# Banus/pano360

Measured on AMD Instinct MI355X. Metric: blended megapixels/sec (multiband), higher is better.
Workload: dtype f32; 1 GPU; cfg3: 32 synthetic 3840x2160 frames per image set, spherical warp + multiband blend L=5, native resolution (MAX_RESOLUTION uncapped); frames=32

## Files before the change

include/pano360.h:

```cpp
#ifndef PANO360_H
#define PANO360_H

#include <stddef.h>
#include <stdint.h>

#ifdef __cplusplus
extern "C" {
#endif

#define PANO_OK 0
#define PANO_EINVAL (-1)
#define PANO_EHIP (-2)
#define PANO_ELIMIT (-3)
#define PANO_ESOLVE (-4)

#define PANO_MAX_TAPS 129
#define PANO_MAX_LEVELS 8
#define PANO_TAP_LEAD 7
#define PANO_TAP_PAD 40
#ifndef PANO_INTERIOR_BLOCK
#define PANO_INTERIOR_BLOCK 4
#endif
#ifndef PANO_MEDIAN_KEEP
#define PANO_MEDIAN_KEEP 32
// ... 84 lines not shown
                        const double *tan_p, const float *lut255, const double *hat_x,
                        const double *hat_y, int gx0, int gy0, int pw, int ph,
                        float *planes, uint8_t *mask, float *map_x, float *map_y);

int pano_warp_windows(pano_ctx *ctx, const pano_camera *cams, const pano_patch *patches,
                      int n, int max_vw, int max_vh, const double *sin_t,
                      const double *cos_t, const double *tan_p, const float *lut,
                      int lut_stride, const uint8_t *need);

int pano_ownership(pano_ctx *ctx, const pano_patch *patches, int n, int H, int W,
                   int16_t *owner, uint8_t *valid);

int pano_ownership_cameras(pano_ctx *ctx, const pano_camera *cams, int n, int H, int W,
                           int xs0, int xs1, const double *sin_t, const double *cos_t,
                           const double *tan_p, int16_t *owner, uint8_t *valid);

int pano_owned_regions(pano_ctx *ctx, const int16_t *owner, int H, int W, int xs0, int xs1,
                       int n, int min_gap, int max_spans, uint8_t *marks,
                       int32_t *regions);

int pano_ownership_regions(pano_ctx *ctx, const pano_camera *cams, int n, int H, int W,
                           int xs0, int xs1, const double *sin_t, const double *cos_t,
                           const double *tan_p, int16_t *owner, uint8_t *valid,
                           int min_gap, int max_spans, uint8_t *marks, int32_t *regions);

int pano_blur_tile_grid(const pano_ctx *ctx);
int pano_blur_tiles(pano_ctx *ctx, const pano_patch *patches, int n, int max_aw,
                    int max_ah, int W, int radius, const uint8_t *interior,
                    uint8_t *tile_flags, uint8_t *warp_need);
int pano_multiband_blur_prepare(pano_ctx *ctx, const pano_patch *patches, int n,
// ... 436 lines not shown
```

pano360_amd/_lib.py:

```python
import ctypes as C
import os
import subprocess

import numpy as np

_HERE = os.path.dirname(os.path.abspath(__file__))
LIB_PATH = os.environ.get("PANO_LIB") or os.path.join(_HERE, "libpano360_hip.so")

MAX_TAPS = 129
MAX_LEVELS = 8
TAP_LEAD = 7
TAP_PAD = 40
OPT_BLUR_KERNEL, OPT_OWN_PRUNE, OPT_BLUR_SEGMENTS, OPT_BLUR_LEAN, OPT_STITCH_STREAMS = 0, 1, 2, 3, 4
OPT_STITCH_ASYNC = 5
OPT_BLUR_SEG_LEN = 6
OPT_SIFT_GRAPH = 7
OPT_LEVEL_CLASSES = 8
BLUR_MFMA, BLUR_VALU = 0, 1


class PanoError(RuntimeError):
    """A C-ABI call returned a negative status."""


# ... 190 lines not shown
    "pano_ctx_destroy": (_i, [_vp]),
    "pano_ctx_set_stream": (_i, [_vp, _vp]),
    "pano_ctx_set_option": (_i, [_vp, _i, _i]),
    "pano_ctx_get_option": (_i, [_vp, _i, C.POINTER(C.c_int)]),
    "pano_timing_enable": (_i, [_vp, _i]),
    "pano_kernel_count": (_i, []),
    "pano_kernel_name": (C.c_char_p, [_i]),
    "pano_timing_read": (_i, [_vp, _i, C.POINTER(C.c_double), C.POINTER(C.c_int)]),
    "pano_add_weights": (_i, [_vp, _vp, _i, _i, _vp, _vp, _vp, _vp]),
    "pano_warp_spherical": (_i, [_vp, _vp, _i, _i, _vp, _vp, _vp, _vp, _vp, _vp, _vp, _i, _i, _i,
                                 _i, _vp, _vp, _vp, _vp]),
    "pano_warp_windows": (_i, [_vp, _vp, _vp, _i, _i, _i, _vp, _vp, _vp, _vp, _i, _vp]),
    "pano_blur_tiles": (_i, [_vp, _vp, _i, _i, _i, _i, _i, _vp, _vp, _vp]),
    "pano_ownership": (_i, [_vp, _vp, _i, _i, _i, _vp, _vp]),
    "pano_ownership_cameras": (_i, [_vp, _vp, _i, _i, _i, _i, _i, _vp, _vp, _vp, _vp, _vp]),
    "pano_owned_regions": (_i, [_vp, _vp, _i, _i, _i, _i, _i, _i, _i, _vp, _vp]),
    "pano_ownership_regions": (_i, [_vp, _vp, _i, _i, _i, _i, _i, _vp, _vp, _vp, _vp, _vp,
                                    _i, _i, _vp, _vp]),
    "pano_multiband_blur": (_i, [_vp, _vp, _i, _i, _i, _i, _vp, _i, _vp, C.POINTER(C.c_int), _i,
                                 _vp, _vp]),
    "pano_multiband_blur_prepare": (_i, [_vp, _vp, _i, _i, _i, _i, _vp, _vp]),
    "pano_layout_windows": (_i, [_i, _vp, _i, _i, _vp, _vp, _i, _i, _i, _i, _vp, _i, _vp]),
    "pano_layout_place": (_i, [_vp, _i, _vp, _vp, _vp]),
    "pano_interior_map": (_i, [_vp, _vp, _i, _i, _i, _i, _i, _vp, _vp]),
    "pano_interior_classes": (_i, [_vp, _vp, _i, _i, _i, _i, _vp, _i, _vp, _vp, _vp]),
    "pano_multiband_compose": (_i, [_vp, _vp, _i, _i, _i, _i, _i, _i, _vp, _vp, _vp, _vp, _vp, _vp,
                                    _vp, _vp, _vp, _i, _vp, _vp]),
    "pano_blend_cameras": (_i, [_vp, _vp, _i, _i, _i, _i, _i, _i, _vp, _vp, _vp, _vp, _i, _vp,
                                _vp]),
    "pano_blur_tile_grid": (_i, [_vp]),
# ... 226 lines not shown
```

pano360_amd/csrc/api.hip:

```cpp
#include <stdarg.h>
#include <stdio.h>
#include <stdlib.h>
#include <string.h>

#include <vector>

#include "common.h"
#include "layout.h"

static thread_local char g_error[512] = "";

void pano_set_error(const char *fmt, ...) {
    va_list ap;
    va_start(ap, fmt);
    vsnprintf(g_error, sizeof(g_error), fmt, ap);
    va_end(ap);
}

extern "C" const char *pano_version(void) { return "pano360_hip 0.1 (gfx950)"; }

extern "C" const char *pano_last_error(void) { return g_error; }

extern "C" int pano_device_count(void) {
    int n = 0;
// ... 127 lines not shown
    PANO_REQUIRE(ctx, "pano_ctx_set_stream: null context");
    if ((hipStream_t)stream != ctx->stream) stitch_memo_void_geometry(ctx->memo);
    ctx->stream = (hipStream_t)stream;
    return PANO_OK;
}

extern "C" int pano_ctx_set_option(pano_ctx *ctx, int option, int value) {
    PANO_REQUIRE(ctx, "pano_ctx_set_option: null context");
    PANO_REQUIRE(option >= 0 && option < PANO_OPT_COUNT, "pano_ctx_set_option: option %d", option);
    if (option == PANO_OPT_BLUR_KERNEL)
        PANO_REQUIRE(value == PANO_BLUR_MFMA || value == PANO_BLUR_VALU,
                     "pano_ctx_set_option: blur kernel %d", value);
    else if (option == PANO_OPT_STITCH_ASYNC)
        PANO_REQUIRE(value >= 0 && value <= 2, "pano_ctx_set_option: option %d takes 0, 1 or 2", option);
    else if (option == PANO_OPT_OWN_PRUNE)
        PANO_REQUIRE(value >= 0 && value <= 3, "pano_ctx_set_option: option %d takes 0 .. 3", option);
    else if (option == PANO_OPT_BLUR_SEG_LEN)
        PANO_REQUIRE(value == -1 || value == 0 || (value >= 4 && value <= 2047),
                     "pano_ctx_set_option: option %d takes -1, 0 or 4 .. 2047", option);
    else
        PANO_REQUIRE(value == 0 || value == 1, "pano_ctx_set_option: option %d takes 0 or 1", option);
    const bool changed = ctx->opt[option] != value;
    ctx->opt[option] = value;
    ctx->prepared_table = ctx->flags_table = ctx->list_table = nullptr;
    stitch_memo_void_geometry(ctx->memo);
    if (changed && option == PANO_OPT_BLUR_KERNEL) stitch_memo_void_layout(ctx->memo);
    return PANO_OK;
}

extern "C" int pano_ctx_get_option(const pano_ctx *ctx, int option, int *value) {
    PANO_REQUIRE(ctx && value, "pano_ctx_get_option: null pointer");
// ... 199 lines not shown
```

pano360_amd/csrc/blend.hip:

```cpp
#include <stdlib.h>

#include "geom.h"

__global__ __launch_bounds__(256) void ownership_kernel(
    const pano_patch *__restrict__ patches, int n, int H, int W,
    int16_t *__restrict__ owner, uint8_t *__restrict__ valid) {
    const int x = blockIdx.x * 64 + threadIdx.x, y = blockIdx.y * 4 + threadIdx.y;
    if (x >= W || y >= H) return;
    float best = 0.0f;
    int who = -1;
    bool any = false;
    for (int i = 0; i < n; ++i) {
        const pano_patch p = patches[i];
        const int px = x - p.x0, py = y - p.y0;
        if ((unsigned)px >= (unsigned)p.w || (unsigned)py >= (unsigned)p.h) continue;
        const float a = p.planes[3 * (size_t)p.vh * p.vpitch + (size_t)py * p.vpitch + px];
        if (a > best) {
            best = a;
            who = i;
        }
        any |= p.mask[(size_t)py * p.w + px] == 0;
    }
    owner[(size_t)y * W + x] = (int16_t)who;
    valid[(size_t)y * W + x] = any ? 1 : 0;
// ... 396 lines not shown
    const int tid = wave * 64 + lane;
    if (tid < listed) {
        const int *b = s_box[tid];
        if (b[1] >= b[0]) box_merge(boxes + (size_t)box_stride * sh.list[tid], b[0], b[1], b[2], b[3]);
    }
}

#define OW_T 64
#define OW_Q 16
#define OW_CAMS 32
#define OW_QLIST 8
#define OW_ILP 4
#define OW_EVAL (-3)
#define OW_NOBODY (-1)
#define OW_UNOWNED (-2)

#define OW_SUBS 8
#define OW_FN(name) name
#include "own_tile.inc"
#undef OW_FN
#define OW_TH_TALL (OW_Q * OW_SUBS)

template <bool LINEAR, bool PERCAM>
__global__ __launch_bounds__(256) void blend_cameras_kernel(
    const pano_camera *__restrict__ cams, int n, int H, int W, int xs0, int xs1,
    const double *__restrict__ sin_t, const double *__restrict__ cos_t,
    const double *__restrict__ tan_p, const float *__restrict__ lut,
    uint8_t *__restrict__ mosaic, uint8_t *__restrict__ valid) {
    __shared__ CamList sh;
    __shared__ CamPrune pr;
// ... 478 lines not shown
#define MOSAIC_GRID dim3 block(64, 4), grid(ceil_div(W, 64), ceil_div(H, 4))

extern "C" int pano_ownership(pano_ctx *ctx, const pano_patch *patches, int n, int H, int W,
                              int16_t *owner, uint8_t *valid) {
    PANO_ENTER(ctx, "pano_ownership");
    if (int rc = check_table(patches, n, H, W, "pano_ownership")) return rc;
    PANO_REQUIRE(owner && valid, "pano_ownership: null output");
    MOSAIC_GRID;
    PANO_TIMED(PK_OWNERSHIP, (hipStream_t)stream,
               hipLaunchKernelGGL(ownership_kernel, grid, block, 0, (hipStream_t)stream,
                                  patches, n, H, W, owner, valid));
    PANO_LAUNCH_CHECK("ownership_kernel");
    return PANO_OK;
}

extern "C" int pano_ownership_cameras(pano_ctx *ctx, const pano_camera *cams, int n, int H, int W,
                                      int xs0, int xs1, const double *sin_t, const double *cos_t,
                                      const double *tan_p, int16_t *owner, uint8_t *valid) {
    PANO_ENTER(ctx, "pano_ownership_cameras");
    if (int rc = check_table(cams, n, H, W, "pano_ownership_cameras")) return rc;
    PANO_REQUIRE(sin_t && cos_t && tan_p && owner && valid, "pano_ownership_cameras: null pointer");
    if (int rc = check_strip(xs0, xs1, W, "pano_ownership_cameras")) return rc;
    if (xs0 == xs1) return PANO_OK;
    const int prune = ctx->opt[PANO_OPT_OWN_PRUNE];
    dim3 block(64, 4), grid(ceil_div(xs1 - xs0, 64), ceil_div(H, (prune & 2) ? OWN_TILE_ROWS : OW_TH_TALL));
    PANO_TIMED(PK_OWNERSHIP_CAMS, (hipStream_t)stream,
               hipLaunchKernelGGL((prune & 2) ? ownership_cameras_l1_kernel : ownership_cameras_kernel,
                                  grid, block, (prune & 2) ? 0 : own_shared_bytes(n),
                                  (hipStream_t)stream, cams, n, H, W, xs0, xs1, sin_t, cos_t,
                                  tan_p, owner, valid, prune & 1, (int32_t *)nullptr, 0,
                                  (uint8_t *)nullptr));
    PANO_LAUNCH_CHECK("ownership_cameras_kernel");
    return PANO_OK;
}

extern "C" int pano_blend_cameras(pano_ctx *ctx, const pano_camera *cams, int n, int H, int W,
                                  int xs0, int xs1, int linear, const double *sin_t,
                                  const double *cos_t, const double *tan_p, const float *lut,
                                  int lut_stride, uint8_t *mosaic, uint8_t *valid) {
    PANO_ENTER(ctx, "pano_blend_cameras");
    if (int rc = check_fused_blend(cams, n, H, W, xs0, xs1, sin_t, cos_t, tan_p, lut, lut_stride,
                                   mosaic, "pano_blend_cameras")) return rc;
    if (xs0 == xs1) return PANO_OK;
    dim3 block(64, 4), grid(ceil_div(xs1 - xs0, 64), ceil_div(H, 4));
    hipStream_t s = (hipStream_t)stream;
#define BLEND(LIN, PC)                                                                        \
    PANO_TIMED(PK_BLEND_CAMERAS, s,                                                           \
               hipLaunchKernelGGL((blend_cameras_kernel<LIN, PC>), grid, block, 0, s, cams, n, \
// ... 118 lines not shown
                                      int xs0, int xs1, const double *sin_t, const double *cos_t,
                                      const double *tan_p, int16_t *owner, uint8_t *valid,
                                      int min_gap, int max_spans, uint8_t *marks,
                                      int32_t *regions) {
    PANO_ENTER(ctx, "pano_ownership_regions");
    if (int rc = check_table(cams, n, H, W, "pano_ownership_regions")) return rc;
    PANO_REQUIRE(sin_t && cos_t && tan_p && owner && valid && marks && regions,
                 "pano_ownership_regions: null pointer");
    if (int rc = check_strip(xs0, xs1, W, "pano_ownership_regions")) return rc;
    PANO_REQUIRE(max_spans >= 1 && min_gap >= 0, "pano_ownership_regions: bad argument");
    if (n == 0) return PANO_OK;
    hipStream_t s = (hipStream_t)stream;
    const int stride = 5 + 2 * max_spans;
    if (int rc = launch_init_regions(s, regions, n, stride, marks, W)) return rc;
    if (xs0 == xs1) return PANO_OK;
    const int prune = ctx->opt[PANO_OPT_OWN_PRUNE];
    dim3 block(64, 4), grid(ceil_div(xs1 - xs0, 64), ceil_div(H, (prune & 2) ? OWN_TILE_ROWS : OW_TH_TALL));
    PANO_TIMED(PK_OWNERSHIP_CAMS, s,
               hipLaunchKernelGGL((prune & 2) ? ownership_cameras_l1_kernel : ownership_cameras_kernel,
                                  grid, block, (prune & 2) ? 0 : own_shared_bytes(n), s, cams, n, H, W, xs0,
                                  xs1, sin_t, cos_t, tan_p, owner, valid, prune & 1, regions, stride,
                                  marks));
    PANO_LAUNCH_CHECK("ownership_cameras_kernel");
    PANO_TIMED(PK_OWNED_SPANS, s,
               hipLaunchKernelGGL(owned_spans_kernel, dim3(n), dim3(256), 0, s, marks, W, xs0, xs1,
                                  min_gap, max_spans, stride, regions));
    PANO_LAUNCH_CHECK("owned_spans_kernel");
    return PANO_OK;
}

static int interior_map_launch(pano_ctx *ctx, const int16_t *owner, int H, int W, int xs0, int xs1,
                               const int *radii, int n_radii, int16_t *block_owner,
                               uint8_t *interior, uint8_t *classes, const char *who) {
    void *const stream = (void *)ctx->stream;
    PANO_REQUIRE(owner && block_owner && interior && radii, "%s: null pointer", who);
    PANO_REQUIRE(H > 0 && W > 0 && n_radii >= 1 && n_radii < PANO_MAX_LEVELS, "%s: bad argument", who);
    if (int rc = check_strip(xs0, xs1, W, who)) return rc;
    LevelReaches lv = {};
// ... 221 lines not shown
```

pano360_amd/csrc/geom.h:

```cpp
#pragma once
#include "common.h"

struct Taps {
    int x0, x1, y0, y1;
    float w00, w01, w10, w11;
};

__device__ __forceinline__ Taps tap_base(float px, float py) {
    int sx = cv_round(px * 32.0f), sy = cv_round(py * 32.0f);
    int fx = sx & 31, fy = sy & 31;
    Taps t;
    t.x0 = sat16(sx >> 5);
    t.y0 = sat16(sy >> 5);
    t.x1 = t.x0 + 1;
    t.y1 = t.y0 + 1;
    float ax = (float)fx * (1.0f / 32.0f), ay = (float)fy * (1.0f / 32.0f);
    t.w00 = (1.0f - ay) * (1.0f - ax);
    t.w01 = (1.0f - ay) * ax;
    t.w10 = ay * (1.0f - ax);
    t.w11 = ay * ax;
    return t;
}

__device__ __forceinline__ void reflect_taps(Taps &t, int sw, int sh) {
// ... 179 lines not shown
    bool m = fz < 0.0f;
    m |= (px < 0.0f) | (px > (float)(sw - 1)) | (py < 0.0f) | (py > (float)(sh - 1));
    return m;
}

__device__ __forceinline__ float alpha_at(const double *__restrict__ hat_x_,
                                          const double *__restrict__ hat_y_,
                                          const Taps &tp) {
    typedef const __attribute__((address_space(1))) double *hat_ptr;
    const hat_ptr hat_x = (hat_ptr)hat_x_, hat_y = (hat_ptr)hat_y_;
    const double hy0 = hat_y[tp.y0], hy1 = hat_y[tp.y1];
    const double hx0 = hat_x[tp.x0], hx1 = hat_x[tp.x1];
    return lerp4((float)(hy0 * hx0), (float)(hy0 * hx1), (float)(hy1 * hx0),
                 (float)(hy1 * hx1), tp);
}
```

pano360_amd/csrc/own_tile.inc:

```
#define OW_TH (OW_Q * OW_SUBS)
#define OW_NQ (4 * OW_SUBS)

struct OW_FN(OwnShared) {
    CamList cl;
    pano_camera cam[OW_CAMS];
    double sn[OW_T], cs[OW_T], tn[OW_TH];
    double rq[4][4];
    double rall[4];
    double step2;
    double rsub[OW_SUBS][2];
    int low1[OW_SUBS], ncand[OW_SUBS];
    int subfill[OW_SUBS];
    float hi2[OW_NQ][OW_QLIST];
    int low2[OW_NQ];
    short qlist[OW_NQ][OW_QLIST];
    int qn[OW_NQ];
    int qfill[OW_NQ];
    int evalq[OW_NQ], n_eval;
    alignas(16) short town[OW_TH][OW_T];
};
static inline size_t OW_FN(own_shared_bytes)(int n) {
    const size_t nl = (size_t)(n < OWN_LIST ? n : OWN_LIST);
    return sizeof(OW_FN(OwnShared)) + nl * (16 + 4 * OW_SUBS + 2 * OW_SUBS) + 16;
}

template <int MODE>
__device__ __forceinline__ void OW_FN(own_tile)(OW_FN(OwnShared) &S, int (*__restrict__ s_box)[4],
                                         float *__restrict__ s_hi, short *__restrict__ s_keep, int NL,
                                         const pano_camera *__restrict__ cams, int n,
                                         int H, int W, int bx0, int bx1, int by0, int by1,
                                         int listed, int prune, int vt, int16_t *__restrict__ owner,
                                         uint8_t *__restrict__ valid, int32_t *__restrict__ boxes,
                                         int box_stride, uint8_t *__restrict__ marks) {
    const int lane = threadIdx.x, wave = threadIdx.y, tid = wave * 64 + lane;
    auto index_at = [&](int pos) -> int { return listed < 0 ? pos : S.cl.list[pos]; };
    auto cam_at = [&](int pos) -> const pano_camera * {
        if (MODE == 1) return &S.cam[pos];
        if (MODE == 2) return &S.cam[index_at(pos)];
        return cams + index_at(pos);
    };

    if (listed == 0) {
        if (tid < OW_NQ) S.qfill[tid] = OW_NOBODY;
// ... 105 lines not shown
                       bx0 + OW_Q * (lane & 3) < bx1;
        const unsigned long long bal = __ballot(e);
        if (e) S.evalq[__popcll(bal & ((1ull << lane) - 1ull))] = lane;
        if (lane == 0) S.n_eval = __popcll(bal);
    }
    __syncthreads();
    constexpr int PER_Q = 4 / OW_ILP;
    const int n_items = PER_Q * S.n_eval;
#pragma unroll 1
    for (int item = wave; item < n_items; item += 4) {
        const int qid = S.evalq[item / PER_Q], sub = qid >> 2, q = qid & 3;
        const int col = OW_Q * q + (lane & (OW_Q - 1));
        const int row0 = OW_Q * sub + 4 * OW_ILP * (item % PER_Q) + (lane >> 4);
        const int xc = min(bx0 + col, bx1 - 1);
        const double s = S.sn[col], c = S.cs[col];
        double t[OW_ILP];
        int y[OW_ILP], who[OW_ILP];
        float best[OW_ILP];
        bool any[OW_ILP];
#pragma unroll
        for (int j = 0; j < OW_ILP; ++j) {
            t[j] = S.tn[row0 + 4 * j];
            y[j] = min(by0 + row0 + 4 * j, by1 - 1);
            best[j] = 0.0f;
            who[j] = -1;
            any[j] = false;
        }
        const int mode = S.qn[qid];
        const int ncand = mode >= 0 ? mode : (mode == -1 ? S.ncand[sub] : (listed < 0 ? n : listed));
        for (int k = 0; k < ncand; ++k) {
            const int pos = __builtin_amdgcn_readfirstlane(
                mode >= 0 ? (int)S.qlist[qid][k] : (mode == -1 ? (int)s_keep[sub * NL + k] : k));
            const pano_camera *cam = cam_at(pos);
            const int i = index_at(pos);
            const int px = xc - cam->x0, sw = cam->sw, sh_ = cam->sh;
            const int cam_y0 = cam->y0, cam_h = cam->h;
            const bool in_x = (unsigned)px < (unsigned)cam->w;
            Taps tp[OW_ILP];
            bool ok[OW_ILP];
#pragma unroll
            for (int j = 0; j < OW_ILP; ++j) {
                float fx, fy;
                const bool m = map_pixel(cam->proj, s, c, t[j], sw, sh_, fx, fy);
                ok[j] = in_x & ((unsigned)(y[j] - cam_y0) < (unsigned)cam_h) & !m;
                tp[j] = make_taps_unmasked(ok[j] ? fx : 0.0f, ok[j] ? fy : 0.0f, sw, sh_);
            }
            typedef const __attribute__((address_space(1))) double *hat_ptr;
            const hat_ptr hat_x = (hat_ptr)cam->hat_x, hat_y = (hat_ptr)cam->hat_y;
            double hx0[OW_ILP], hx1[OW_ILP], hy0[OW_ILP], hy1[OW_ILP];
#pragma unroll
            for (int j = 0; j < OW_ILP; ++j) {
                hy0[j] = hat_y[tp[j].y0];
                hy1[j] = hat_y[tp[j].y1];
                hx0[j] = hat_x[tp[j].x0];
                hx1[j] = hat_x[tp[j].x1];
            }
#pragma unroll
            for (int j = 0; j < OW_ILP; ++j) {
                const float a = lerp4((float)(hy0[j] * hx0[j]), (float)(hy0[j] * hx1[j]),
                                      (float)(hy1[j] * hx0[j]), (float)(hy1[j] * hx1[j]), tp[j]);
                any[j] |= ok[j];
                const bool wins = ok[j] & (a > best[j]);
                best[j] = wins ? a : best[j];
                who[j] = wins ? i : who[j];
            }
        }
#pragma unroll
        for (int j = 0; j < OW_ILP; ++j)
            S.town[row0 + 4 * j][col] = (short)(who[j] >= 0 ? who[j] : (any[j] ? OW_UNOWNED : OW_NOBODY));
    }
    __syncthreads();
    const int rows = by1 - by0, ncols = min(bx1 - bx0, OW_T);
    typedef short short8 __attribute__((ext_vector_type(8)));
    typedef short8 short8_any __attribute__((aligned(2)));
    typedef unsigned int uint2v __attribute__((ext_vector_type(2)));
    typedef uint2v uint2_any __attribute__((aligned(1)));
#pragma unroll
    for (int k = 0; k < OW_TH / 32; ++k) {
        const int row = 32 * k + 8 * wave + (lane >> 3), c0 = 8 * (lane & 7);
        if (row >= rows || c0 >= ncols) continue;
        const int fill = S.qfill[(row >> 4) * 4 + (c0 >> 4)];
        short8 w8 = (short)fill;
        if (fill == OW_EVAL) w8 = *(const short8 *)&S.town[row][c0];
        short8 own8;
        unsigned char ok8[8];
#pragma unroll
// ... 63 lines not shown
                    run_o = w;
                    run_y0 = y;
                }
                run_y1 = y;
            }
            flush(run_o, run_y0, run_y1);
        }
    }
    __syncthreads();
    if (n <= OWN_LIST && tid < n) {
        const int *b = s_box[tid];
        if (b[1] >= b[0]) box_merge(boxes + (size_t)box_stride * tid, b[0], b[1], b[2], b[3]);
    }
}

__global__ __launch_bounds__(256) void OW_FN(ownership_cameras_kernel)(
    const pano_camera *__restrict__ cams, int n, int H, int W, int xs0, int xs1,
    const double *__restrict__ sin_t, const double *__restrict__ cos_t,
    const double *__restrict__ tan_p, int16_t *__restrict__ owner,
    uint8_t *__restrict__ valid, int prune, int32_t *__restrict__ boxes, int box_stride,
    uint8_t *__restrict__ marks) {
    extern __shared__ __align__(16) unsigned char own_smem[];
    OW_FN(OwnShared) &S = *(OW_FN(OwnShared) *)own_smem;
    const int NL = min(n, OWN_LIST);
    int (*s_box)[4] = (int (*)[4])(own_smem + ((sizeof(OW_FN(OwnShared)) + 15) & ~(size_t)15));
    float *s_hi = (float *)(s_box + NL);
    short *s_keep = (short *)(s_hi + OW_SUBS * NL);
    const int lane = threadIdx.x, wave = threadIdx.y, tid = wave * 64 + lane;
    const int bx0 = xs0 + blockIdx.x * OW_T, by0 = blockIdx.y * OW_TH;
    const int bx1 = min(bx0 + OW_T, xs1), by1 = min(by0 + OW_TH, H);
    const int vt = (tid + 64 * (int)((blockIdx.x + blockIdx.y) & 3)) & 255;
    if (marks && tid < NL) {
        int *b = s_box[tid];
        b[0] = b[2] = 0x7fffffff;
        b[1] = b[3] = -1;
    }
    constexpr int DW = (int)(sizeof(pano_camera) / 4);
    const bool all_cams = n <= OW_CAMS;
    uint32_t rec_dw[(OW_CAMS * DW + 255) / 256];
    if (all_cams) {
#pragma unroll
        for (int r = 0; r < (OW_CAMS * DW + 255) / 256; ++r) {
// ... 52 lines not shown
            S.tn[64 * r + lane] = trow[r];
            double lo_t = trow[r], hi_t = trow[r];
#pragma unroll
            for (int off = 1; off < OW_Q; off <<= 1) {
                lo_t = fmin(lo_t, __shfl_xor(lo_t, off, 64));
                hi_t = fmax(hi_t, __shfl_xor(hi_t, off, 64));
            }
            if ((lane & (OW_Q - 1)) == 0)
                S.rsub[4 * r + lane / OW_Q][0] = lo_t, S.rsub[4 * r + lane / OW_Q][1] = hi_t;
        }
    } else if (wave == 2 && lane < OW_NQ) {
        S.low2[lane] = 0;
        S.qn[lane] = -2;
        S.qfill[lane] = OW_EVAL;
        if (lane < OW_SUBS) S.low1[lane] = 0, S.ncand[lane] = 0;
    }
    __syncthreads();
#define OW_CALL(M)                                                                                  \
    OW_FN(own_tile)<M>(S, s_box, s_hi, s_keep, NL, cams, n, H, W, bx0, bx1, by0, by1, listed, prune, vt,  \
                owner, valid, boxes, box_stride, marks)
    if (mode == 2)
        OW_CALL(2);
    else if (mode == 1)
        OW_CALL(1);
    else
        OW_CALL(0);
#undef OW_CALL
}


#undef OW_TH
#undef OW_NQ
```

pano360_amd/engine.py:

```python
import collections
import ctypes as C

import numpy as np

from . import _lib
from ._lib import Patch, _ptr

BORDER_SAMPLES = 100
MULTIBAND_PAD = 10
VerifiedStitch = collections.namedtuple("VerifiedStitch", "signature plan patches owner valid")


class SphProj:

    @staticmethod
    def hom2proj(pts):
        pts = np.asarray(pts)
        xz = np.sqrt(pts[:, 0] ** 2 + pts[:, 2] ** 2)
        theta = np.arctan2(pts[:, 0], pts[:, 2])
        phi = np.arctan2(pts[:, 1], xz)
        return np.stack([theta, phi], axis=-1)

    @staticmethod
    def proj2hom(pts):
# ... 481 lines not shown
        self.lib = _lib.lib()
        if not torch.cuda.is_available() or self.lib.pano_device_count() < 1:
            raise _lib.PanoError("no MI355X visible: the HIP path has no CPU fallback")
        self.device = torch.device(device if device is not None
                                   else f"cuda:{torch.cuda.current_device()}")
        index = self.device.index if self.device.index is not None else torch.cuda.current_device()
        self.device = torch.device("cuda", index)
        self._device_index = index
        handle = C.c_void_p()
        self._ctx_stream = torch.cuda.current_stream(self.device).cuda_stream
        _lib.call("pano_ctx_create", index, self._ctx_stream, C.byref(handle))
        self._ctx = handle
        if blur not in ("mfma", "valu"):
            raise ValueError(f"blur kernel {blur!r}: 'mfma' or 'valu'")
        self.set_option(_lib.OPT_BLUR_KERNEL, _lib.BLUR_VALU if blur == "valu" else _lib.BLUR_MFMA)
        self.set_option(_lib.OPT_OWN_PRUNE, 1 if own_prune else 0)
        self.tile_grid = int(self.lib.pano_blur_tile_grid(self._ctx))
        self.interior_block = int(self.lib.pano_interior_block())
        lut = np.arange(256, dtype=np.float32) / np.float32(255)
        self.lut255 = torch.from_numpy(lut).to(self.device)
        self._hats = {}
        self._taps = {}
        self._region_bufs = {}
        self._arenas = {}
        self._ring = None
        self.warp_need = "auto"
        self._cam_template = None
        self.native_stitch = True
        self._stitch_ws = {}
        self._plans = PlanMemo()
        self.trust_layout = False
# ... 374 lines not shown
        return dev

    def ownership_cameras(self, plan, strip=None, out=None, cams=None):
        torch = _torch()
        H, W = plan.shape
        if out is None:
            owner = torch.empty((H, W), dtype=torch.int16, device=self.device)
            valid = torch.empty((H, W), dtype=torch.uint8, device=self.device)
        else:
            owner, valid = out
        xs0, xs1 = strip if strip is not None else (0, W)
        if cams is None:
            cams = self.camera_table(plan)
        self.call("pano_ownership_cameras", cams, plan.n, H, W, xs0, xs1, *plan.dev, owner, valid)
        return owner, valid

    def ownership_regions(self, plan, strip=None, min_gap=0, max_spans=4, cams=None):
        torch = _torch()
        H, W = plan.shape
        owner = torch.empty((H, W), dtype=torch.int16, device=self.device)
        valid = torch.empty((H, W), dtype=torch.uint8, device=self.device)
        marks = torch.empty((plan.n, W), dtype=torch.uint8, device=self.device)
        regions = torch.empty((plan.n, 5 + 2 * max_spans), dtype=torch.int32, device=self.device)
        xs0, xs1 = strip if strip is not None else (0, W)
        if cams is None:
            cams = self.camera_table(plan)
        self.call("pano_ownership_regions", cams, plan.n, H, W, xs0, xs1, *plan.dev, owner, valid,
                  min_gap, max_spans, marks, regions)
        return owner, valid, regions, marks

# ... 315 lines not shown
```

Baseline: 203,100 MP/s.

## Screen ownership candidates with fp32 error bounds before exact double-precision evaluation

Adds an fp32 screening pass to the ownership kernel. Each candidate camera's pixel is classified as in, out or unsure using rigorous rounding-error bounds and bilinear-weight bounds. Pixels whose winner is decided are written directly, and only ambiguous pixels are queued in a shared-memory list for the exact double-precision hat-weight evaluation. This is meant to cut the costly double map_pixel and hat-table lookups. In exchange it adds shared memory, a second pass with divergence, and a risk of mismatches if the bounds are not conservative. It also adds a counting variant of the kernel for diagnostics and sets launch bounds to 4 blocks.

```diff
diff --git a/include/pano360.h b/include/pano360.h
--- a/include/pano360.h
+++ b/include/pano360.h
@@ -122,6 +122,11 @@
 int pano_ownership_cameras(pano_ctx *ctx, const pano_camera *cams, int n, int H, int W,
                            int xs0, int xs1, const double *sin_t, const double *cos_t,
                            const double *tan_p, int16_t *owner, uint8_t *valid);
+
+int pano_ownership_screen_counts(pano_ctx *ctx, const pano_camera *cams, int n, int H, int W,
+                                 int xs0, int xs1, const double *sin_t, const double *cos_t,
+                                 const double *tan_p, int16_t *owner, uint8_t *valid,
+                                 int64_t *counts);
 
 int pano_owned_regions(pano_ctx *ctx, const int16_t *owner, int H, int W, int xs0, int xs1,
                        int n, int min_gap, int max_spans, uint8_t *marks,
diff --git a/pano360_amd/_lib.py b/pano360_amd/_lib.py
--- a/pano360_amd/_lib.py
+++ b/pano360_amd/_lib.py
@@ -228,6 +228,7 @@
     "pano_blur_tiles": (_i, [_vp, _vp, _i, _i, _i, _i, _i, _vp, _vp, _vp]),
     "pano_ownership": (_i, [_vp, _vp, _i, _i, _i, _vp, _vp]),
     "pano_ownership_cameras": (_i, [_vp, _vp, _i, _i, _i, _i, _i, _vp, _vp, _vp, _vp, _vp]),
+    "pano_ownership_screen_counts": (_i, [_vp, _vp, _i, _i, _i, _i, _i, _vp, _vp, _vp, _vp, _vp, _vp]),
     "pano_owned_regions": (_i, [_vp, _vp, _i, _i, _i, _i, _i, _i, _i, _vp, _vp]),
     "pano_ownership_regions": (_i, [_vp, _vp, _i, _i, _i, _i, _i, _vp, _vp, _vp, _vp, _vp,
                                     _i, _i, _vp, _vp]),
diff --git a/pano360_amd/csrc/api.hip b/pano360_amd/csrc/api.hip
--- a/pano360_amd/csrc/api.hip
+++ b/pano360_amd/csrc/api.hip
@@ -165,7 +165,7 @@
     else if (option == PANO_OPT_STITCH_ASYNC)
         PANO_REQUIRE(value >= 0 && value <= 2, "pano_ctx_set_option: option %d takes 0, 1 or 2", option);
     else if (option == PANO_OPT_OWN_PRUNE)
-        PANO_REQUIRE(value >= 0 && value <= 3, "pano_ctx_set_option: option %d takes 0 .. 3", option);
+        PANO_REQUIRE(value >= 0 && value <= 15, "pano_ctx_set_option: option %d takes 0 .. 15", option);
     else if (option == PANO_OPT_BLUR_SEG_LEN)
         PANO_REQUIRE(value == -1 || value == 0 || (value >= 4 && value <= 2047),
                      "pano_ctx_set_option: option %d takes -1, 0 or 4 .. 2047", option);
diff --git a/pano360_amd/csrc/blend.hip b/pano360_amd/csrc/blend.hip
--- a/pano360_amd/csrc/blend.hip
+++ b/pano360_amd/csrc/blend.hip
@@ -434,6 +434,9 @@
 #define OW_EVAL (-3)
 #define OW_NOBODY (-1)
 #define OW_UNOWNED (-2)
+#define OW_LCAP 2048
+#define OW_LCAP_SMALL 6
+#define OW_LIST_VOID 0xffffu
 
 #define OW_SUBS 8
 #define OW_FN(name) name
@@ -942,6 +945,32 @@
     return PANO_OK;
 }
 
+static int launch_ownership_cameras(pano_ctx *ctx, hipStream_t s, const pano_camera *cams, int n, int H,
+                                    int W, int xs0, int xs1, const double *sin_t, const double *cos_t,
+                                    const double *tan_p, int16_t *owner, uint8_t *valid, int32_t *boxes,
+                                    int box_stride, uint8_t *marks, unsigned long long *counts) {
+    const int prune = ctx->opt[PANO_OPT_OWN_PRUNE];
+    dim3 block(64, 4), grid(ceil_div(xs1 - xs0, 64), ceil_div(H, (prune & 2) ? OWN_TILE_ROWS : OW_TH_TALL));
+    if (counts) {
+        PANO_REQUIRE(!(prune & 2), "pano_ownership_screen_counts: the one-level kernel does not screen");
+        hipLaunchKernelGGL(ownership_cameras_count_kernel, grid, block, own_shared_bytes(n), s, cams, n, H,
+                           W, xs0, xs1, sin_t, cos_t, tan_p, owner, valid, prune & 13, boxes, box_stride,
+                           marks, counts);
+    } else if (prune & 2) {
+        PANO_TIMED(PK_OWNERSHIP_CAMS, s,
+                   hipLaunchKernelGGL(ownership_cameras_l1_kernel, grid, block, 0, s, cams, n, H, W, xs0,
+                                      xs1, sin_t, cos_t, tan_p, owner, valid, prune & 1, boxes,
+                                      box_stride, marks));
+    } else {
+        PANO_TIMED(PK_OWNERSHIP_CAMS, s,
+                   hipLaunchKernelGGL(ownership_cameras_kernel, grid, block, own_shared_bytes(n), s, cams,
+                                      n, H, W, xs0, xs1, sin_t, cos_t, tan_p, owner, valid, prune & 13,
+                                      boxes, box_stride, marks));
+    }
+    PANO_LAUNCH_CHECK("ownership_cameras_kernel");
+    return PANO_OK;
+}
+
 extern "C" int pano_ownership_cameras(pano_ctx *ctx, const pano_camera *cams, int n, int H, int W,
                                       int xs0, int xs1, const double *sin_t, const double *cos_t,
                                       const double *tan_p, int16_t *owner, uint8_t *valid) {
@@ -950,16 +979,23 @@
     PANO_REQUIRE(sin_t && cos_t && tan_p && owner && valid, "pano_ownership_cameras: null pointer");
     if (int rc = check_strip(xs0, xs1, W, "pano_ownership_cameras")) return rc;
     if (xs0 == xs1) return PANO_OK;
-    const int prune = ctx->opt[PANO_OPT_OWN_PRUNE];
-    dim3 block(64, 4), grid(ceil_div(xs1 - xs0, 64), ceil_div(H, (prune & 2) ? OWN_TILE_ROWS : OW_TH_TALL));
-    PANO_TIMED(PK_OWNERSHIP_CAMS, (hipStream_t)stream,
-               hipLaunchKernelGGL((prune & 2) ? ownership_cameras_l1_kernel : ownership_cameras_kernel,
-                                  grid, block, (prune & 2) ? 0 : own_shared_bytes(n),
-                                  (hipStream_t)stream, cams, n, H, W, xs0, xs1, sin_t, cos_t,
-                                  tan_p, owner, valid, prune & 1, (int32_t *)nullptr, 0,
-                                  (uint8_t *)nullptr));
-    PANO_LAUNCH_CHECK("ownership_cameras_kernel");
-    return PANO_OK;
+    return launch_ownership_cameras(ctx, (hipStream_t)stream, cams, n, H, W, xs0, xs1, sin_t, cos_t, tan_p,
+                                    owner, valid, nullptr, 0, nullptr, nullptr);
+}
+
+extern "C" int pano_ownership_screen_counts(pano_ctx *ctx, const pano_camera *cams, int n, int H, int W,
+                                            int xs0, int xs1, const double *sin_t, const double *cos_t,
+                                            const double *tan_p, int16_t *owner, uint8_t *valid,
+                                            int64_t *counts) {
+    PANO_ENTER(ctx, "pano_ownership_screen_counts");
+    if (int rc = check_table(cams, n, H, W, "pano_ownership_screen_counts")) return rc;
+    PANO_REQUIRE(sin_t && cos_t && tan_p && owner && valid && counts,
+                 "pano_ownership_screen_counts: null pointer");
+    if (int rc = check_strip(xs0, xs1, W, "pano_ownership_screen_counts")) return rc;
+    PANO_HIP(hipMemsetAsync(counts, 0, 4 * sizeof(int64_t), (hipStream_t)stream));
+    if (xs0 == xs1) return PANO_OK;
+    return launch_ownership_cameras(ctx, (hipStream_t)stream, cams, n, H, W, xs0, xs1, sin_t, cos_t, tan_p,
+                                    owner, valid, nullptr, 0, nullptr, (unsigned long long *)counts);
 }
 
 extern "C" int pano_blend_cameras(pano_ctx *ctx, const pano_camera *cams, int n, int H, int W,
@@ -1108,14 +1144,8 @@
     const int stride = 5 + 2 * max_spans;
     if (int rc = launch_init_regions(s, regions, n, stride, marks, W)) return rc;
     if (xs0 == xs1) return PANO_OK;
-    const int prune = ctx->opt[PANO_OPT_OWN_PRUNE];
-    dim3 block(64, 4), grid(ceil_div(xs1 - xs0, 64), ceil_div(H, (prune & 2) ? OWN_TILE_ROWS : OW_TH_TALL));
-    PANO_TIMED(PK_OWNERSHIP_CAMS, s,
-               hipLaunchKernelGGL((prune & 2) ? ownership_cameras_l1_kernel : ownership_cameras_kernel,
-                                  grid, block, (prune & 2) ? 0 : own_shared_bytes(n), s, cams, n, H, W, xs0,
-                                  xs1, sin_t, cos_t, tan_p, owner, valid, prune & 1, regions, stride,
-                                  marks));
-    PANO_LAUNCH_CHECK("ownership_cameras_kernel");
+    if (int rc = launch_ownership_cameras(ctx, s, cams, n, H, W, xs0, xs1, sin_t, cos_t, tan_p, owner, valid,
+                                          regions, stride, marks, nullptr)) return rc;
     PANO_TIMED(PK_OWNED_SPANS, s,
                hipLaunchKernelGGL(owned_spans_kernel, dim3(n), dim3(256), 0, s, marks, W, xs0, xs1,
                                   min_gap, max_spans, stride, regions));
diff --git a/pano360_amd/csrc/geom.h b/pano360_amd/csrc/geom.h
--- a/pano360_amd/csrc/geom.h
+++ b/pano360_amd/csrc/geom.h
@@ -217,3 +217,61 @@
     return lerp4((float)(hy0 * hx0), (float)(hy0 * hx1), (float)(hy1 * hx0),
                  (float)(hy1 * hx1), tp);
 }
+
+struct OwnScreenCam {
+    float ax, ay, az;
+    float mx, my, mz;
+    float k1, k4, k7;
+    float limx, limy;
+    float isw, ish;
+    float kx, ky;
+    float rx, ry;
+};
+#define OWN_SCREEN_U 1.1920929e-7f
+enum { OWN_SCREEN_OUT = 0, OWN_SCREEN_IN = 1, OWN_SCREEN_UNSURE = 2 };
+
+__device__ __forceinline__ OwnScreenCam own_screen_cam(const double *K, int sw, int sh, float sf, float cf) {
+    const float u8 = 8.0f * OWN_SCREEN_U;
+    OwnScreenCam o;
+    const float k0 = (float)K[0], k2 = (float)K[2], k3 = (float)K[3], k5 = (float)K[5];
+    const float k6 = (float)K[6], k8 = (float)K[8];
+    o.k1 = (float)K[1], o.k4 = (float)K[4], o.k7 = (float)K[7];
+    o.ax = fmaf(k2, cf, k0 * sf);
+    o.ay = fmaf(k5, cf, k3 * sf);
+    o.az = fmaf(k8, cf, k6 * sf);
+    o.mx = u8 * (fabsf(k0 * sf) + fabsf(k2 * cf));
+    o.my = u8 * (fabsf(k3 * sf) + fabsf(k5 * cf));
+    o.mz = u8 * (fabsf(k6 * sf) + fabsf(k8 * cf)) + 1e-30f;
+    const float fw = (float)sw, fh = (float)sh;
+    o.limx = 0.5f * fw - 0.5f, o.limy = 0.5f * fh - 0.5f;
+    o.isw = __builtin_amdgcn_rcpf(fw), o.ish = __builtin_amdgcn_rcpf(fh);
+    o.kx = (sw & 1) ? 0.5f * o.isw : 0.0f;
+    o.ky = (sh & 1) ? 0.5f * o.ish : 0.0f;
+    o.rx = u8 * (0.5f * fw), o.ry = u8 * (0.5f * fh);
+    return o;
+}
+
+__device__ __forceinline__ int own_screen_pixel(const OwnScreenCam &o, float tf, float ta8, float &lo,
+                                                float &hi) {
+    const float u8 = 8.0f * OWN_SCREEN_U;
+    const float vx = fmaf(o.k1, tf, o.ax), vy = fmaf(o.k4, tf, o.ay), vz = fmaf(o.k7, tf, o.az);
+    const float ex = fmaf(fabsf(o.k1), ta8, o.mx), ey = fmaf(fabsf(o.k4), ta8, o.my);
+    const float ez = fmaf(fabsf(o.k7), ta8, o.mz);
+    const float rz = __builtin_amdgcn_rcpf(vz);
+    const float qx = vx * rz, qy = vy * rz, aqx = fabsf(qx), aqy = fabsf(qy);
+    const float rz11 = rz * 1.1f;
+    const float epx = fmaf(fmaf(aqx, ez, ex), rz11, fmaf(u8, aqx, o.rx));
+    const float epy = fmaf(fmaf(aqy, ez, ey), rz11, fmaf(u8, aqy, o.ry));
+    const float bx = fabsf(qx + 0.5f), by = fabsf(qy + 0.5f);
+    const bool front = vz >= 16.0f * ez;
+    const bool in = front & (bx < o.limx - epx) & (by < o.limy - epy);
+    const bool out = (vz < -4.0f * ez) | (front & ((bx > o.limx + epx) | (by > o.limy + epy)));
+    const float hx = fmaf(-aqx, o.isw, 0.5f), hy = fmaf(-aqy, o.ish, 0.5f);
+    float dx = fmaf(epx + 1.0f / 64.0f, o.isw, 4.0f * OWN_SCREEN_U);
+    float dy = fmaf(epy + 1.0f / 64.0f, o.ish, 4.0f * OWN_SCREEN_U);
+    dx = aqx < 1.02f + epx ? dx + o.kx : dx;
+    dy = aqy < 1.02f + epy ? dy + o.ky : dy;
+    lo = fmaxf(hx - dx, 0.0f) * fmaxf(hy - dy, 0.0f) * (1.0f - 16.0f * OWN_SCREEN_U);
+    hi = (hx + dx) * (hy + dy) * (1.0f + 16.0f * OWN_SCREEN_U);
+    return in ? OWN_SCREEN_IN : (out ? OWN_SCREEN_OUT : OWN_SCREEN_UNSURE);
+}
diff --git a/pano360_amd/csrc/own_tile.inc b/pano360_amd/csrc/own_tile.inc
--- a/pano360_amd/csrc/own_tile.inc
+++ b/pano360_amd/csrc/own_tile.inc
@@ -21,12 +21,52 @@
 };
 static inline size_t OW_FN(own_shared_bytes)(int n) {
     const size_t nl = (size_t)(n < OWN_LIST ? n : OWN_LIST);
-    return sizeof(OW_FN(OwnShared)) + nl * (16 + 4 * OW_SUBS + 2 * OW_SUBS) + 16;
+    return sizeof(OW_FN(OwnShared)) + nl * (16 + 4 * OW_SUBS + 2 * OW_SUBS) + 16 + 4 + 32 + 2 * OW_LCAP;
 }
 
-template <int MODE>
+template <int ILP>
+__device__ __forceinline__ void OW_FN(own_exact_cam)(const pano_camera *cam, int i, int xc, double s, double c,
+                                                     const double (&t)[ILP], const int (&y)[ILP],
+                                                     float (&best)[ILP], int (&who)[ILP], bool (&any)[ILP],
+                                                     bool live) {
+    const int px = xc - cam->x0, sw = cam->sw, sh_ = cam->sh;
+    const int cam_y0 = cam->y0, cam_h = cam->h;
+    const bool in_x = live & ((unsigned)px < (unsigned)cam->w);
+    Taps tp[ILP];
+    bool ok[ILP];
+#pragma unroll
+    for (int j = 0; j < ILP; ++j) {
+        float fx, fy;
+        const bool m = map_pixel(cam->proj, s, c, t[j], sw, sh_, fx, fy);
+        ok[j] = in_x & ((unsigned)(y[j] - cam_y0) < (unsigned)cam_h) & !m;
+        tp[j] = make_taps_unmasked(ok[j] ? fx : 0.0f, ok[j] ? fy : 0.0f, sw, sh_);
+    }
+    typedef const __attribute__((address_space(1))) double *hat_ptr;
+    const hat_ptr hat_x = (hat_ptr)cam->hat_x, hat_y = (hat_ptr)cam->hat_y;
+    double hx0[ILP], hx1[ILP], hy0[ILP], hy1[ILP];
+#pragma unroll
+    for (int j = 0; j < ILP; ++j) {
+        hy0[j] = hat_y[tp[j].y0];
+        hy1[j] = hat_y[tp[j].y1];
+        hx0[j] = hat_x[tp[j].x0];
+        hx1[j] = hat_x[tp[j].x1];
+    }
+#pragma unroll
+    for (int j = 0; j < ILP; ++j) {
+        const float a = lerp4((float)(hy0[j] * hx0[j]), (float)(hy0[j] * hx1[j]),
+                              (float)(hy1[j] * hx0[j]), (float)(hy1[j] * hx1[j]), tp[j]);
+        any[j] |= ok[j];
+        const bool wins = ok[j] & (a > best[j]);
+        best[j] = wins ? a : best[j];
+        who[j] = wins ? i : who[j];
+    }
+}
+
+template <int MODE, bool COUNT>
 __device__ __forceinline__ void OW_FN(own_tile)(OW_FN(OwnShared) &S, int (*__restrict__ s_box)[4],
                                          float *__restrict__ s_hi, short *__restrict__ s_keep, int NL,
+                                         int *__restrict__ s_lhead, unsigned short *__restrict__ s_ulist,
+                                         bool screen, int lcap, unsigned long long *__restrict__ counts,
                                          const pano_camera *__restrict__ cams, int n,
                                          int H, int W, int bx0, int bx1, int by0, int by1,
                                          int listed, int prune, int vt, int16_t *__restrict__ owner,
@@ -162,62 +202,131 @@
         const int row0 = OW_Q * sub + 4 * OW_ILP * (item % PER_Q) + (lane >> 4);
         const int xc = min(bx0 + col, bx1 - 1);
         const double s = S.sn[col], c = S.cs[col];
-        double t[OW_ILP];
-        int y[OW_ILP], who[OW_ILP];
-        float best[OW_ILP];
-        bool any[OW_ILP];
-#pragma unroll
-        for (int j = 0; j < OW_ILP; ++j) {
-            t[j] = S.tn[row0 + 4 * j];
-            y[j] = min(by0 + row0 + 4 * j, by1 - 1);
-            best[j] = 0.0f;
-            who[j] = -1;
-            any[j] = false;
-        }
         const int mode = S.qn[qid];
         const int ncand = mode >= 0 ? mode : (mode == -1 ? S.ncand[sub] : (listed < 0 ? n : listed));
-        for (int k = 0; k < ncand; ++k) {
-            const int pos = __builtin_amdgcn_readfirstlane(
+        auto pos_at = [&](int k) -> int {
+            return __builtin_amdgcn_readfirstlane(
                 mode >= 0 ? (int)S.qlist[qid][k] : (mode == -1 ? (int)s_keep[sub * NL + k] : k));
-            const pano_camera *cam = cam_at(pos);
-            const int i = index_at(pos);
-            const int px = xc - cam->x0, sw = cam->sw, sh_ = cam->sh;
-            const int cam_y0 = cam->y0, cam_h = cam->h;
-            const bool in_x = (unsigned)px < (unsigned)cam->w;
-            Taps tp[OW_ILP];
-            bool ok[OW_ILP];
+        };
+        bool whole = !screen;
+        if (screen) {
+            const float sf = (float)s, cf = (float)c;
+            float tf[OW_ILP], ta8[OW_ILP], blo[OW_ILP], bhi[OW_ILP], rest[OW_ILP];
+            int who[OW_ILP];
+            const int y0 = by0 + row0;
 #pragma unroll
             for (int j = 0; j < OW_ILP; ++j) {
-                float fx, fy;
-                const bool m = map_pixel(cam->proj, s, c, t[j], sw, sh_, fx, fy);
-                ok[j] = in_x & ((unsigned)(y[j] - cam_y0) < (unsigned)cam_h) & !m;
-                tp[j] = make_taps_unmasked(ok[j] ? fx : 0.0f, ok[j] ? fy : 0.0f, sw, sh_);
-            }
-            typedef const __attribute__((address_space(1))) double *hat_ptr;
-            const hat_ptr hat_x = (hat_ptr)cam->hat_x, hat_y = (hat_ptr)cam->hat_y;
-            double hx0[OW_ILP], hx1[OW_ILP], hy0[OW_ILP], hy1[OW_ILP];
+                tf[j] = (float)S.tn[row0 + 4 * j];
+                ta8[j] = 8.0f * OWN_SCREEN_U * fabsf(tf[j]);
+                blo[j] = -1.0f;
+                bhi[j] = rest[j] = 0.0f;
+                who[j] = OW_NOBODY;
+            }
+            for (int k = 0; k < ncand; ++k) {
+                const int pos = pos_at(k);
+                const pano_camera *cam = cam_at(pos);
+                const int i = index_at(pos);
+                const int dy0 = y0 - cam->y0, cam_h = cam->h;
+                const bool in_x = (unsigned)(xc - cam->x0) < (unsigned)cam->w;
+                const OwnScreenCam sc = own_screen_cam(cam->proj, cam->sw, cam->sh, sf, cf);
+#pragma unroll
+                for (int j = 0; j < OW_ILP; ++j) {
+                    float lo, hi;
+                    const int st = own_screen_pixel(sc, tf[j], ta8[j], lo, hi);
+                    const bool cand = in_x & ((unsigned)(dy0 + 4 * j) < (unsigned)cam_h);
+                    const bool in = cand & (st == OWN_SCREEN_IN), unsure = cand & (st == OWN_SCREEN_UNSURE);
+                    const bool take = in & (lo > blo[j]);
+                    rest[j] = fmaxf(rest[j], unsure ? __builtin_inff() : in ? (take ? bhi[j] : hi) : 0.0f);
+                    blo[j] = take ? lo : blo[j];
+                    bhi[j] = take ? hi : bhi[j];
+                    who[j] = take ? i : who[j];
+                }
+            }
+            unsigned long long bal[OW_ILP];
+            int cnt = 0, inside = 0;
 #pragma unroll
             for (int j = 0; j < OW_ILP; ++j) {
-                hy0[j] = hat_y[tp[j].y0];
-                hy1[j] = hat_y[tp[j].y1];
-                hx0[j] = hat_x[tp[j].x0];
-                hx1[j] = hat_x[tp[j].x1];
-            }
+                const bool here = (bx0 + col < bx1) & (y0 + 4 * j < by1);
+                const bool und = here & !((blo[j] > rest[j]) | ((blo[j] < 0.0f) & (rest[j] <= 0.0f)));
+                bal[j] = __ballot(und);
+                cnt += __popcll(bal[j]);
+                if (COUNT) inside += __popcll(__ballot(here));
+            }
+            int base = 0;
+            if (cnt > 0) {
+                if (lane == 0) base = atomicAdd(&s_lhead[0], cnt);
+                base = __builtin_amdgcn_readfirstlane(base);
+            }
+            whole = base + cnt > lcap;
+            if (COUNT && lane == 0) {
+                atomicAdd(&s_lhead[1], inside);
+                atomicAdd(&s_lhead[whole ? 3 : 2], whole ? 1 : cnt);
+            }
+            if (!whole) {
+                int at = base;
+#pragma unroll
+                for (int j = 0; j < OW_ILP; ++j) {
+                    S.town[row0 + 4 * j][col] = (short)who[j];
+                    if (bal[j] >> lane & 1ull)
+                        s_ulist[at + __popcll(bal[j] & ((1ull << lane) - 1ull))] =
+                            (unsigned short)((row0 + 4 * j) << 6 | col);
+                    at += __popcll(bal[j]);
+                }
+            } else {
+                for (int e = base + lane; e < min(base + cnt, lcap); e += 64) s_ulist[e] = OW_LIST_VOID;
+            }
+        }
+        if (whole) {
+            double t[OW_ILP];
+            int y[OW_ILP], who[OW_ILP];
+            float best[OW_ILP];
+            bool any[OW_ILP];
 #pragma unroll
             for (int j = 0; j < OW_ILP; ++j) {
-                const float a = lerp4((float)(hy0[j] * hx0[j]), (float)(hy0[j] * hx1[j]),
-                                      (float)(hy1[j] * hx0[j]), (float)(hy1[j] * hx1[j]), tp[j]);
-                any[j] |= ok[j];
-                const bool wins = ok[j] & (a > best[j]);
-                best[j] = wins ? a : best[j];
-                who[j] = wins ? i : who[j];
-            }
-        }
-#pragma unroll
-        for (int j = 0; j < OW_ILP; ++j)
-            S.town[row0 + 4 * j][col] = (short)(who[j] >= 0 ? who[j] : (any[j] ? OW_UNOWNED : OW_NOBODY));
+                t[j] = S.tn[row0 + 4 * j];
+                y[j] = min(by0 + row0 + 4 * j, by1 - 1);
+                best[j] = 0.0f;
+                who[j] = -1;
+                any[j] = false;
+            }
+            for (int k = 0; k < ncand; ++k) {
+                const int pos = pos_at(k);
+                OW_FN(own_exact_cam)<OW_ILP>(cam_at(pos), index_at(pos), xc, s, c, t, y, best, who, any, true);
+            }
+#pragma unroll
+            for (int j = 0; j < OW_ILP; ++j)
+                S.town[row0 + 4 * j][col] = (short)(who[j] >= 0 ? who[j] : (any[j] ? OW_UNOWNED : OW_NOBODY));
+        }
+    }
+    if (screen) {
+        __syncthreads();
+        const int nl = min(s_lhead[0], lcap);
+#pragma unroll 1
+        for (int base = 64 * wave; base < nl; base += 256) {
+            const int e = base + lane < nl ? (int)s_ulist[base + lane] : (int)OW_LIST_VOID;
+            const bool act = e != (int)OW_LIST_VOID;
+            const int row = act ? e >> 6 : 0, col = act ? e & 63 : 0;
+            const int sub = row >> 4, qid = sub * 4 + (col >> 4);
+            const int mode = S.qn[qid];
+            const int nc = !act ? 0 : mode >= 0 ? mode : (mode == -1 ? S.ncand[sub] : (listed < 0 ? n : listed));
+            const int xc = min(bx0 + col, bx1 - 1);
+            const double s = S.sn[col], c = S.cs[col];
+            const double t[1] = {S.tn[row]};
+            const int y[1] = {min(by0 + row, by1 - 1)};
+            float best[1] = {0.0f};
+            int who[1] = {-1};
+            bool any[1] = {false};
+            for (int k = 0; __ballot(k < nc) != 0ull; ++k) {
+                const bool live = k < nc;
+                const int pos = !live ? 0 : mode >= 0 ? (int)S.qlist[qid][k] : (mode == -1 ? (int)s_keep[sub * NL + k] : k);
+                OW_FN(own_exact_cam)<1>(cam_at(pos), index_at(pos), xc, s, c, t, y, best, who, any, live);
+            }
+            if (act) S.town[row][col] = (short)(who[0] >= 0 ? who[0] : (any[0] ? OW_UNOWNED : OW_NOBODY));
+            if (COUNT && lane == 0) atomicAdd(&s_lhead[4], 1);
+        }
     }
     __syncthreads();
+    if (COUNT && tid < 4) atomicAdd(counts + tid, (unsigned long long)s_lhead[1 + tid]);
     const int rows = by1 - by0, ncols = min(bx1 - bx0, OW_T);
     typedef short short8 __attribute__((ext_vector_type(8)));
     typedef short8 short8_any __attribute__((aligned(2)));
@@ -311,18 +420,23 @@
     }
 }
 
-__global__ __launch_bounds__(256) void OW_FN(ownership_cameras_kernel)(
+template <bool COUNT>
+__device__ __forceinline__ void OW_FN(own_kernel_body)(unsigned char *__restrict__ own_smem,
     const pano_camera *__restrict__ cams, int n, int H, int W, int xs0, int xs1,
     const double *__restrict__ sin_t, const double *__restrict__ cos_t,
     const double *__restrict__ tan_p, int16_t *__restrict__ owner,
     uint8_t *__restrict__ valid, int prune, int32_t *__restrict__ boxes, int box_stride,
-    uint8_t *__restrict__ marks) {
-    extern __shared__ __align__(16) unsigned char own_smem[];
+    uint8_t *__restrict__ marks, unsigned long long *__restrict__ counts) {
     OW_FN(OwnShared) &S = *(OW_FN(OwnShared) *)own_smem;
     const int NL = min(n, OWN_LIST);
     int (*s_box)[4] = (int (*)[4])(own_smem + ((sizeof(OW_FN(OwnShared)) + 15) & ~(size_t)15));
     float *s_hi = (float *)(s_box + NL);
     short *s_keep = (short *)(s_hi + OW_SUBS * NL);
+    int *s_lhead = (int *)(((uintptr_t)(s_keep + OW_SUBS * NL) + 3) & ~(uintptr_t)3);
+    unsigned short *s_ulist = (unsigned short *)(s_lhead + 8);
+    const bool screen = !(prune & 4);
+    const int lcap = (prune & 8) ? OW_LCAP_SMALL : OW_LCAP;
+    prune &= 1;
     const int lane = threadIdx.x, wave = threadIdx.y, tid = wave * 64 + lane;
     const int bx0 = xs0 + blockIdx.x * OW_T, by0 = blockIdx.y * OW_TH;
     const int bx1 = min(bx0 + OW_T, xs1), by1 = min(by0 + OW_TH, H);
@@ -405,11 +519,13 @@
         S.qn[lane] = -2;
         S.qfill[lane] = OW_EVAL;
         if (lane < OW_SUBS) S.low1[lane] = 0, S.ncand[lane] = 0;
+    } else if (wave == 3 && lane < 8) {
+        s_lhead[lane] = 0;
     }
     __syncthreads();
 #define OW_CALL(M)                                                                                  \
-    OW_FN(own_tile)<M>(S, s_box, s_hi, s_keep, NL, cams, n, H, W, bx0, bx1, by0, by1, listed, prune, vt,  \
-                owner, valid, boxes, box_stride, marks)
+    OW_FN(own_tile)<M, COUNT>(S, s_box, s_hi, s_keep, NL, s_lhead, s_ulist, screen, lcap, counts, cams, n,  \
+                       H, W, bx0, bx1, by0, by1, listed, prune, vt, owner, valid, boxes, box_stride, marks)
     if (mode == 2)
         OW_CALL(2);
     else if (mode == 1)
@@ -419,6 +535,23 @@
 #undef OW_CALL
 }
 
+#define OW_KERNEL_ARGS                                                                              \
+    const pano_camera *__restrict__ cams, int n, int H, int W, int xs0, int xs1,                    \
+    const double *__restrict__ sin_t, const double *__restrict__ cos_t,                             \
+    const double *__restrict__ tan_p, int16_t *__restrict__ owner, uint8_t *__restrict__ valid,     \
+    int prune, int32_t *__restrict__ boxes, int box_stride, uint8_t *__restrict__ marks
+__global__ __launch_bounds__(256, 4) void OW_FN(ownership_cameras_kernel)(OW_KERNEL_ARGS) {
+    extern __shared__ __align__(16) unsigned char own_smem[];
+    OW_FN(own_kernel_body)<false>(own_smem, cams, n, H, W, xs0, xs1, sin_t, cos_t, tan_p, owner, valid, prune,
+                                  boxes, box_stride, marks, nullptr);
+}
+__global__ __launch_bounds__(256, 4) void OW_FN(ownership_cameras_count_kernel)(
+    OW_KERNEL_ARGS, unsigned long long *__restrict__ counts) {
+    extern __shared__ __align__(16) unsigned char own_smem[];
+    OW_FN(own_kernel_body)<true>(own_smem, cams, n, H, W, xs0, xs1, sin_t, cos_t, tan_p, owner, valid, prune,
+                                 boxes, box_stride, marks, counts);
+}
+#undef OW_KERNEL_ARGS
 
 #undef OW_TH
 #undef OW_NQ
diff --git a/pano360_amd/engine.py b/pano360_amd/engine.py
--- a/pano360_amd/engine.py
+++ b/pano360_amd/engine.py
@@ -1,5 +1,6 @@
 import collections
 import ctypes as C
+import os
 
 import numpy as np
 
@@ -519,7 +520,8 @@
         if blur not in ("mfma", "valu"):
             raise ValueError(f"blur kernel {blur!r}: 'mfma' or 'valu'")
         self.set_option(_lib.OPT_BLUR_KERNEL, _lib.BLUR_VALU if blur == "valu" else _lib.BLUR_MFMA)
-        self.set_option(_lib.OPT_OWN_PRUNE, 1 if own_prune else 0)
+        self.set_option(_lib.OPT_OWN_PRUNE, (1 if own_prune else 0)
+                        | (4 if os.environ.get("PANO_OWN_SCREEN") == "0" else 0))
         self.tile_grid = int(self.lib.pano_blur_tile_grid(self._ctx))
         self.interior_block = int(self.lib.pano_interior_block())
         lut = np.arange(256, dtype=np.float32) / np.float32(255)
@@ -924,6 +926,19 @@
             cams = self.camera_table(plan)
         self.call("pano_ownership_cameras", cams, plan.n, H, W, xs0, xs1, *plan.dev, owner, valid)
         return owner, valid
+
+    def ownership_screen_counts(self, plan, strip=None, cams=None):
+        torch = _torch()
+        H, W = plan.shape
+        owner = torch.empty((H, W), dtype=torch.int16, device=self.device)
+        valid = torch.empty((H, W), dtype=torch.uint8, device=self.device)
+        counts = torch.empty(4, dtype=torch.int64, device=self.device)
+        xs0, xs1 = strip if strip is not None else (0, W)
+        if cams is None:
+            cams = self.camera_table(plan)
+        self.call("pano_ownership_screen_counts", cams, plan.n, H, W, xs0, xs1, *plan.dev, owner, valid,
+                  counts)
+        return owner, valid, counts.cpu().numpy()
 
     def ownership_regions(self, plan, strip=None, min_gap=0, max_spans=4, cams=None):
         torch = _torch()
```

Result: no change. 204,300 MP/s (median of 6 runs) (+0.6%).
